# JasonTStanley/MultiDroneSim

Measured on AMD Instinct MI355X. Metric: drone-steps/sec (whole node) at N_envs×N_drones; achieved HBM GB/s vs roofline, higher is better.
Workload: dtype f32

## Files before the change

include/mds.h:

```cpp
#ifndef MDS_H
#define MDS_H

#include <stddef.h>
#include <stdint.h>

#ifdef __cplusplus
extern "C" {
#endif

#define MDS_VERSION 202
#define MDS_OBS_DIM 20
#define MDS_ACT_DIM 4
#define MDS_STATE_DIM 13
#define MDS_DES_DIM 11
#define MDS_LEM_DIM 7
#define MDS_GEO_AUX_DIM 13

typedef enum mds_status {
  MDS_OK = 0,
  MDS_EINVAL = -1,
  MDS_ENOMEM = -2,
  MDS_EHIP = -3,
  MDS_EALIGN = -4,
  MDS_ESTATE = -5,
// ... 34 lines not shown
const char* mds_last_error(void);

int mds_default_config(int drone_model, mds_config* cfg);
int mds_default_geometric_gains(mds_geometric_gains* gains);

int mds_create(const mds_config* cfg, mds_handle** out);
int mds_destroy(mds_handle* h);

int mds_get_derived(const mds_handle* h, double out[8]);

int mds_reset(mds_handle* h, const double* xyz_host, const double* rpy_host, void* stream);

int mds_state_ptrs(mds_handle* h, void* comp_dev[13], size_t stride_elems[13], void* origin_dev[3]);

int mds_get_state(mds_handle* h, double* state_host, void* stream);
int mds_set_state(mds_handle* h, const double* state_host, void* stream);

int mds_set_origin(mds_handle* h, const double* origin_host, void* stream);

int mds_get_obs(mds_handle* h, void* obs_dev, void* stream);

int mds_step(mds_handle* h, const void* action_dev, void* obs_dev, void* stream);

int mds_set_wind(mds_handle* h, const double force_world[3]);

#define MDS_SEG_DIM 40
int mds_set_trajectory_segments(mds_handle* h, const double* segs_host, const int32_t* offsets_host,
                                const int32_t* compound_host, const double* anchor_host, int32_t total_segments, void* stream);
int mds_traj_eval(mds_handle* h, double t, void* des_dev, void* stream);

int mds_set_lemniscate(mds_handle* h, const double* params_host, void* stream);
int mds_traj_yaw_free(mds_handle* h);
int mds_set_traj_specialisation(mds_handle* h, int on);
int mds_set_geometric_gains(mds_handle* h, const mds_geometric_gains* gains);

int mds_step_geometric(mds_handle* h, double t, void* obs_dev, void* action_dev, void* stream);

int mds_rollout_geometric(mds_handle* h, double t0, int n_steps, void* obs_dev, int obs_every_step, void* stream);

int mds_rollout_step(mds_handle* h, const void* actions_dev, int n_action_sets, int first_step, int n_steps, void* obs_log_dev,
                     int log_slots, int episode_len, void* stream);
int mds_rollout_step_fused(mds_handle* h, const void* actions_dev, int n_action_sets, int first_step, int n_steps, void* obs_log_dev,
                           int log_slots, int episode_len, int steps_per_launch, void* stream);
int mds_reset_async(mds_handle* h, void* stream);

typedef struct mds_episode_params {
  int32_t max_steps;
  int32_t reserved;
  double z_min, z_max, max_dist, max_tilt, max_speed, max_rate;
  double reward_r0, term_penalty;
} mds_episode_params;
int mds_default_episode_params(mds_episode_params* params);
int mds_set_episodes(mds_handle* h, const mds_episode_params* params, const double* target_host, void* stream);
int mds_rollout_episodes(mds_handle* h, const void* actions_dev, int n_action_sets, int first_step, int n_steps, void* obs_log_dev,
                         int log_slots, void* reward_log_dev, int32_t* flags_log_dev, int steps_per_launch, void* obs_dev, void* stream);
int mds_step_episodes(mds_handle* h, const void* action_dev, void* obs_dev, void* final_obs_dev, void* reward_dev, int32_t* flags_dev,
                      void* stream);
int mds_episode_ptrs(mds_handle* h, void* ptrs[5]);

#define MDS_EPISODE_MAX_OBSTACLES 16
typedef struct mds_episode_safety {
  double safety_radius, zscale;
  int32_t n_obs, reserved;
} mds_episode_safety;
int mds_set_episode_safety(mds_handle* h, const mds_episode_safety* params, const double* obstacles_host, void* stream);
int mds_episode_safety_ptrs(mds_handle* h, void* ptrs[2]);
// ... 137 lines not shown
```

multidronesim_amd/_capi.py:

```python
from __future__ import annotations

import ctypes as C
import os

_HERE = os.path.dirname(os.path.abspath(__file__))
LIB_PATH = os.environ.get("MDS_LIB_PATH") or os.path.join(_HERE, "libmds.so")

MDS_OK = 0
MDS_F32, MDS_F64, MDS_F16, MDS_F32C = 0, 1, 2, 3
MDS_PHYSICS_DYN, MDS_PHYSICS_DYN_DRAG, MDS_PHYSICS_DYN_GND, MDS_PHYSICS_DYN_DW, MDS_PHYSICS_DYN_GND_DRAG_DW = 0, 1, 2, 3, 4
MDS_INTEGRATOR_EULER, MDS_INTEGRATOR_RK4 = 0, 1
MDS_CF2X, MDS_CF2P = 0, 1
OBS_DIM, ACT_DIM, STATE_DIM, DES_DIM, LEM_DIM, GEO_AUX_DIM, SEG_DIM = 20, 4, 13, 11, 7, 13, 40


class MdsConfig(C.Structure):
    _fields_ = [("num_envs", C.c_int32), ("num_drones", C.c_int32), ("dtype", C.c_int32), ("physics", C.c_int32),
                ("integrator", C.c_int32), ("drone_model", C.c_int32), ("pyb_freq", C.c_int32),
                ("ctrl_freq", C.c_int32), ("device", C.c_int32), ("track_last_rpm", C.c_int32),
                ("M", C.c_double), ("L", C.c_double), ("KF", C.c_double), ("KM", C.c_double), ("J", C.c_double * 3),
                ("G", C.c_double), ("thrust2weight", C.c_double), ("drag_coeff", C.c_double * 3)]


class MdsGeometricGains(C.Structure):
# ... 26 lines not shown
class MdsEpisodeRandomisation(C.Structure):
    _fields_ = [("seed", C.c_uint64), ("first_env", C.c_int64)] + [(k, C.c_double * 3) for k in ("pos", "rpy", "vel", "rate")]


class MdsError(RuntimeError):
    def __init__(self, status, where, detail):
        super().__init__(f"{where}: {detail} (mds_status {status})")
        self.status = status


_P = C.c_void_p
_PD = C.POINTER(C.c_double)

PROTOTYPES = {
    "mds_version": (C.c_int, []),
    "mds_strerror": (C.c_char_p, [C.c_int]),
    "mds_last_error": (C.c_char_p, []),
    "mds_default_config": (C.c_int, [C.c_int, C.POINTER(MdsConfig)]),
    "mds_default_geometric_gains": (C.c_int, [C.POINTER(MdsGeometricGains)]),
    "mds_create": (C.c_int, [C.POINTER(MdsConfig), C.POINTER(_P)]),
    "mds_destroy": (C.c_int, [_P]),
    "mds_get_derived": (C.c_int, [_P, _PD]),
    "mds_reset": (C.c_int, [_P, _PD, _PD, _P]),
    "mds_state_ptrs": (C.c_int, [_P, C.POINTER(C.c_void_p), C.POINTER(C.c_size_t), C.POINTER(C.c_void_p)]),
    "mds_get_state": (C.c_int, [_P, _PD, _P]),
    "mds_set_state": (C.c_int, [_P, _PD, _P]),
    "mds_set_origin": (C.c_int, [_P, _PD, _P]),
    "mds_get_obs": (C.c_int, [_P, _P, _P]),
    "mds_step": (C.c_int, [_P, _P, _P, _P]),
    "mds_set_wind": (C.c_int, [_P, _PD]),
    "mds_set_lemniscate": (C.c_int, [_P, _PD, _P]),
    "mds_traj_yaw_free": (C.c_int, [_P]),
    "mds_set_traj_specialisation": (C.c_int, [_P, C.c_int]),
    "mds_set_trajectory_segments": (C.c_int, [_P, _PD, C.POINTER(C.c_int32), C.POINTER(C.c_int32), _PD, C.c_int32, _P]),
    "mds_traj_eval": (C.c_int, [_P, C.c_double, _P, _P]),
    "mds_set_geometric_gains": (C.c_int, [_P, C.POINTER(MdsGeometricGains)]),
    "mds_step_geometric": (C.c_int, [_P, C.c_double, _P, _P, _P]),
    "mds_rollout_geometric": (C.c_int, [_P, C.c_double, C.c_int, _P, C.c_int, _P]),
    "mds_set_rollout_streams": (C.c_int, [_P, C.c_int]),
    "mds_get_last_rollout_streams": (C.c_int, [_P]),
    "mds_rollout_streams_for": (C.c_int, [_P, C.c_int, C.c_int]),
    "mds_set_rollout_form": (C.c_int, [_P, C.c_int, C.c_int]),
    "mds_rollout_form_for": (C.c_int, [_P, C.c_int]),
    "mds_get_last_rollout_form": (C.c_int, [_P]),
    "mds_rollout_step": (C.c_int, [_P, _P, C.c_int, C.c_int, C.c_int, _P, C.c_int, C.c_int, _P]),
    "mds_rollout_step_fused": (C.c_int, [_P, _P, C.c_int, C.c_int, C.c_int, _P, C.c_int, C.c_int, C.c_int, _P]),
    "mds_reset_async": (C.c_int, [_P, _P]),
    "mds_default_episode_params": (C.c_int, [C.POINTER(MdsEpisodeParams)]),
    "mds_set_episodes": (C.c_int, [_P, C.POINTER(MdsEpisodeParams), _PD, _P]),
    "mds_rollout_episodes": (C.c_int, [_P, _P, C.c_int, C.c_int, C.c_int, _P, C.c_int, _P, _P, C.c_int, _P, _P]),
    "mds_step_episodes": (C.c_int, [_P, _P, _P, _P, _P, _P, _P]),
    "mds_episode_ptrs": (C.c_int, [_P, C.POINTER(C.c_void_p)]),
    "mds_set_episode_safety": (C.c_int, [_P, C.POINTER(MdsEpisodeSafety), _PD, _P]),
    "mds_episode_safety_ptrs": (C.c_int, [_P, C.POINTER(C.c_void_p)]),
    "mds_set_episode_randomisation": (C.c_int, [_P, C.POINTER(MdsEpisodeRandomisation), _P]),
    "mds_reset_episodes": (C.c_int, [_P, _P, _P]),
    "mds_rollout_geometric_fused": (C.c_int, [_P, C.c_double, C.c_int, _P, _P, _P]),
    "mds_lemniscate_eval": (C.c_int, [_P, C.c_double, _P, _P]),
    "mds_geometric_compute": (C.c_int, [_P, _P, _P, _P, _P, _P]),
    "mds_input_to_action": (C.c_int, [_P, _P, _P, _P]),
    "mds_action_to_input": (C.c_int, [_P, _P, C.c_int, _P, _P]),
    "mds_obs_to_model": (C.c_int, [_P, _P, C.c_int, _P, _P]),
    "mds_quadrotor_dynamics": (C.c_int, [C.c_int, C.c_int, _P, _P, C.c_double, _PD, C.c_double, _P, _P]),
    "mds_compare_models": (C.c_int, [_P, C.c_int, _P, _PD, _PD, C.c_double, C.c_double, _PD, C.c_double, _P, _P, _P, _P]),
    "mds_linear_xdot": (C.c_int, [_P, C.c_int, _P, _P, _PD, _PD, C.c_double, _P, _P]),
    "mds_rpy_to_rot": (C.c_int, [C.c_int, C.c_int, _P, _P, _P]),
# ... 102 lines not shown
```

multidronesim_amd/csrc/mds_api.hip:

```cpp
#include <hip/hip_runtime.h>
#include <math.h>
#include <stdio.h>
#include <stdlib.h>
#include <string.h>

#include <new>
#include <type_traits>
#include <unordered_map>
#include <vector>

#include "../../include/mds.h"
#include "mds_consts.hpp"
#include "mds_devmem.hpp"
#include "mds_kernels.hip"
#include "mds_traj_image.hpp"
#ifndef MDS_PART
#define MDS_PART 3
#endif
#if MDS_PART & 1
#include "mds_episode_kernels.hip"
#endif
#if MDS_PART & 2
#include "mds_cbf_kernels.hip"
#include "mds_fedce_kernels.hip"
// ... 73 lines not shown


}

template <typename T> struct HostParams {
  Consts<T> c;
  EnvFx<T> fx;
  CbfParams<T> cbf;
  DslPidGains<T> pid;
  LqrGain<T> lqr;
  LqrYoGain<T> lqr_yo;
  Lqr12Gain<T> lqr12;
};

struct mds_handle {
  explicit mds_handle(const DevAllocator& a) : mem(a) {}
  DevMem mem;
  mds_config cfg = {};
  mds_geometric_gains gains = {};
  double wind[3] = {0.0, 0.0, 0.0};
  int n = 0;
  size_t ld = 0;
  void* state = nullptr;
  void* state_lo = nullptr;
  void* origin = nullptr;
  void* last_rpm = nullptr;
  void* lem = nullptr;
  double* scratch = nullptr;
  double* init_pose = nullptr;
  bool has_traj = false;
  int traj_mode = 0;
  bool traj_yaw_free = false;
  bool traj_spec = true;
  double* segs = nullptr;
  int nseg_total = 0;
  int* tinfo = nullptr;
  HostParams<float> p32 = {};
  HostParams<double> p64 = {};
  bool has_cbf = false;
  mds_cbf_params cbf = {};
  int* pair_ij = nullptr;
  void* obstacles = nullptr;
  int* cbf_order = nullptr;
  int* cbf_count = nullptr;
  int cbf_calls_half[2] = {-1, -1};
  int* cbf_cost = nullptr;
  int cbf_calls = -1;
  int rollout_streams = 0;
  hipStream_t split_st = nullptr;
  hipEvent_t split_ev[2] = {nullptr, nullptr};
  int last_rollout_streams = 0;
  int rollout_form = 0;
  int rollout_chunk = 50;
  int last_rollout_form = 0;
  bool next_nom_ok[3] = {false, false, false};
  double next_nom_t[3] = {0.0, 0.0, 0.0};
  bool cbf_hildreth = false;
  bool cbf_q4 = false;
  int cbf_last_step_kernel = -1;
  bool cbf_step_persistent = false;
  bool cbf_fused = false;
  void* cbf_unom = nullptr;
  void* cbf_xdes = nullptr;
  void* cbf_usafe = nullptr;
  void* ll = nullptr;
  void* pid = nullptr;
// ... 586 lines not shown

int step_env_ctrl(mds_handle* h, int ctrl, double t, const void* u_in, double thrust_offset, void* obs, void* act, hipStream_t st) {
  const dim3 grid = grid_for(h->n, kBlock);
  const int K = h->cfg.pyb_freq / h->cfg.ctrl_freq, D = h->cfg.num_drones;
  void* rpm = rpm_track(h);
  void* abuf = K > 1 ? h->act_scratch : nullptr;
  const void* gain = ctrl == 1 ? h->gain_dev[0] : nullptr;
  with_dtype_no_half(h->cfg.dtype, [&](auto DT) {
    using T = typename decltype(DT)::T;
    with_int<0, 1, 2, 3>(ctrl, [&](auto CTRL) {
      with_flags([&](auto DRAG) {
        k_step_ctrl_env<T, T, DRAG(), CTRL()><<<grid, kBlock, 0, st>>>(params<T>(h).c, params<T>(h).fx, gain, h->n, h->ld, D, t, h->traj_mode,
                                                                       (const T*)h->state, (T*)h->state_alt, (const T*)h->origin, (const T*)h->lem,
                                                                       SegTable{h->segs, h->nseg_total}, h->tinfo, (T*)rpm, (T*)h->ll, (const T*)u_in,
                                                                       (T)(1.0 / h->cfg.ctrl_freq), (T)thrust_offset, (T*)abuf, (T*)obs, (T*)act, K == 1);
      }, has_drag(h));
    });
  });
  MDS_HIP(hipGetLastError());
  void* home = h->state;
  void* tmp = h->state; h->state = h->state_alt; h->state_alt = tmp;
  if (K > 1) return step_env_plain(h, h->act_scratch, obs, st, 1, home);
  return envfx_return_home(h, home, st);
}

int mds_step(mds_handle* h, const void* action, void* obs, void* stream) {
  MDS_DEV(h);
  if (!h || !action) return fail(MDS_EINVAL, "mds_step: null argument");
  if (!aligned16(action) || !aligned16(obs)) return fail(MDS_EALIGN, "mds_step: action_dev/obs_dev");
  if (int rc = step_plain(h, action, obs, Chain{(hipStream_t)stream, 0, 0})) return rc;
  return check_launches();
}

int mds_set_lemniscate(mds_handle* h, const double* params, void* stream) {
  MDS_DEV(h);
  if (!h || !params) return fail(MDS_EINVAL, "mds_set_lemniscate: null argument");
  hipStream_t st = (hipStream_t)stream;
  const int n = h->n;
  double* centres = new (std::nothrow) double[(size_t)n * 3];
  if (!centres) return fail(MDS_ENOMEM, "mds_set_lemniscate: host allocation");
  bool yaw_free = true;
  for (int i = 0; i < n; ++i) {
    for (int k = 0; k < 3; ++k) centres[(size_t)3 * i + k] = params[(size_t)7 * i + 2 + k];
    yaw_free = yaw_free && params[(size_t)7 * i + 5] == 0.0;
  }
  int rc = mds_set_origin(h, centres, stream);
  delete[] centres;
  if (rc != MDS_OK) return rc;
  MDS_HIP(hipMemcpyAsync(h->scratch, params, (size_t)n * 7 * sizeof(double), hipMemcpyHostToDevice, st));
  with_dtype(h->cfg.dtype, [&](auto DT) {
    using T = typename decltype(DT)::T;
    k_set_planes<T><<<grid_for(n, 256), 256, 0, st>>>(n, h->ld, 7, h->scratch, (T*)h->lem);
  });
  MDS_HIP(hipGetLastError());
  MDS_HIP(hipStreamSynchronize(st));
  h->has_traj = true;
  h->traj_mode = 1;
  h->traj_yaw_free = yaw_free;
  return MDS_OK;
}

int mds_traj_yaw_free(mds_handle* h) { return h && h->traj_yaw_free ? 1 : 0; }

int mds_set_traj_specialisation(mds_handle* h, int on) {
  if (!h) return fail(MDS_EINVAL, "mds_set_traj_specialisation: null handle");
  h->traj_spec = on != 0;
  return MDS_OK;
}

static bool use_yaw_free(const mds_handle* h) { return h->traj_mode == 1 && h->traj_yaw_free && h->traj_spec; }

int mds_set_trajectory_segments(mds_handle* h, const double* segs, const int32_t* offsets, const int32_t* compound,
                                const double* anchor, int32_t total, void* stream) {
  MDS_DEV(h);
  if (!h || !segs || !offsets || !compound || !anchor) return fail(MDS_EINVAL, "mds_set_trajectory_segments: null argument");
  const int n = h->n;
  std::vector<int> ti;
  std::vector<double> fm;
  int nu = 0;
  const char* why = "";
  const int brc = build_traj_image(segs, offsets, compound, n, total, fm, ti, nu, &why);
  if (brc != MDS_OK) return fail(brc, why);
  if (int rc = h->mem.alloc(&h->tinfo, sizeof(int) * 3 * n)) return rc;
  const int rc = h->mem.replace(&h->segs, sizeof(double) * fm.size(), [&](void* new_segs) -> int {
    MDS_HIP(hipMemcpy(new_segs, fm.data(), sizeof(double) * fm.size(), hipMemcpyHostToDevice));
    if (int orc = mds_set_origin(h, anchor, stream)) return orc;
    MDS_HIP(hipMemcpy(h->tinfo, ti.data(), sizeof(int) * 3 * n, hipMemcpyHostToDevice));
    return MDS_OK;
  });
  if (rc != MDS_OK) return rc;
  h->nseg_total = nu;
  h->has_traj = true;
  h->traj_mode = 2;
  h->traj_yaw_free = false;
  return MDS_OK;
}

int mds_traj_eval(mds_handle* h, double t, void* des, void* stream) {
  MDS_DEV(h);
  if (!h || !des) return fail(MDS_EINVAL, "mds_traj_eval: null argument");
  if (h->traj_mode == 1) return mds_lemniscate_eval(h, t, des, stream);
  if (h->traj_mode != 2) return fail(MDS_ESTATE, "mds_traj_eval: no trajectories set");
  hipStream_t st = (hipStream_t)stream;
  with_dtype(h->cfg.dtype, [&](auto DT) {
    using S = typename decltype(DT)::S;
    k_traj_eval<S><<<grid_for(h->n, 256), 256, 0, st>>>(h->n, t, SegTable{h->segs, h->nseg_total}, h->tinfo, (S*)des);
  });
  MDS_HIP(hipGetLastError());
  return MDS_OK;
}

int mds_set_geometric_gains(mds_handle* h, const mds_geometric_gains* g) {
  if (!h || !g) return fail(MDS_EINVAL, "mds_set_geometric_gains: null argument");
  if (!(g->max_tilt_angle > 0) || !(g->max_tilt_angle < M_PI / 2)) return fail(MDS_EINVAL, "mds_set_geometric_gains: max_tilt_angle");
  h->gains = *g;
  refill_consts(h);
  return MDS_OK;
}

int mds_set_wind(mds_handle* h, const double force_world[3]) {
  if (!h || !force_world) return fail(MDS_EINVAL, "mds_set_wind: null argument");
  for (int k = 0; k < 3; ++k) h->wind[k] = force_world[k];
  refill_consts(h);
  return MDS_OK;
}

static int step_geometric(mds_handle* h, double t, void* obs, void* act, const Chain& ch) {
// ... 6 lines not shown
  const bool rk4 = h->cfg.integrator == MDS_INTEGRATOR_RK4, drag = has_drag(h);
  if (h->traj_mode == 2) {
    with_flags([&](auto RK4, auto DRAG) {
      with_dtype(h->cfg.dtype, [&](auto DT) {
        using T = typename decltype(DT)::T; using S = typename decltype(DT)::S;
        k_step_traj<T, S, RK4(), DRAG(), DT.COMP><<<grid, kBlock, pad, st>>>(params<T>(h).c, h->n, h->ld, t, (S*)h->state, (const T*)h->origin,
                                                                             SegTable{h->segs, h->nseg_total}, h->tinfo, (T*)rpm_track(h), (S*)obs,
                                                                             (S*)act, (int)batch0, (S*)h->state_lo);
      });
    }, rk4, drag);
    return MDS_OK;
  }
  with_flags([&](auto Y0, auto HAS_OBS, auto HAS_ACT, auto RK4, auto DRAG) {
    with_dtype(h->cfg.dtype, [&](auto DT) {
      using T = typename decltype(DT)::T; using S = typename decltype(DT)::S;
      auto* const k = Y0() ? &k_step_geometric_y0<T, S, HAS_OBS(), HAS_ACT(), RK4(), DRAG(), DT.COMP>
                           : &k_step_geometric<T, S, HAS_OBS(), HAS_ACT(), RK4(), DRAG(), DT.COMP>;
      k<<<grid, kBlock, pad, st>>>(params<T>(h).c, h->n, h->ld, t, (S*)h->state, (const T*)h->lem, (T*)rpm_track(h), (S*)obs, (S*)act, (int)batch0,
                                   (S*)h->state_lo);
    });
  }, use_yaw_free(h), obs != nullptr, act != nullptr, rk4, drag);
  return MDS_OK;
}

int mds_step_geometric(mds_handle* h, double t, void* obs, void* act, void* stream) {
  MDS_DEV(h);
  if (!h) return fail(MDS_EINVAL, "mds_step_geometric: null handle");
  if (!h->has_traj) return fail(MDS_ESTATE, "mds_step_geometric: call mds_set_lemniscate first");
  if (!aligned16(obs) || !aligned16(act)) return fail(MDS_EALIGN, "mds_step_geometric: obs_dev/action_dev");
  if (int rc = step_geometric(h, t, obs, act, Chain{(hipStream_t)stream, 0, 0})) return rc;
  return check_launches();
}

static void launch_rollout_kernel(mds_handle* h, int ctrl, double t0, int n_steps, void* obs_log, size_t log_stride, void* obs_last, hipStream_t st) {
  const dim3 grid = grid_for(h->n, kBlock);
  const double dt = 1.0 / h->cfg.ctrl_freq;
  const int omode = obs_log == nullptr ? kObsLast : log_stride == 0 ? kObsInPlace : kObsLog;
  auto launch = [&](auto DT, auto CTRL) {
    using T = typename decltype(DT)::T; using S = typename decltype(DT)::S;
    constexpr int COMP = DT.COMP ? 1 : 0;
    const void* gain = nullptr;
    if constexpr (CTRL() >= 1) gain = h->gain_dev[CTRL() - 1];
    with_flags([&](auto RK4, auto DRAG) {
      auto roll = [&](auto OBS) {
        if (h->traj_mode == 2) {
          if constexpr (CTRL() <= 1)
            k_rollout_traj<T, S, RK4(), DRAG(), CTRL(), COMP, OBS()><<<grid, kBlock, 0, st>>>(
                params<T>(h).c, gain, h->n, h->ld, t0, dt, n_steps, (S*)h->state, (const T*)h->origin, SegTable{h->segs, h->nseg_total}, h->tinfo,
                (T*)rpm_track(h), (S*)obs_log, log_stride, (S*)obs_last, (S*)h->state_lo);
        } else {
          auto* k = &k_rollout_geometric<T, S, RK4(), DRAG(), CTRL(), COMP, OBS()>;
          if constexpr (CTRL() == 0)
            if (use_yaw_free(h)) k = &k_rollout_geometric_y0<T, S, RK4(), DRAG(), COMP, OBS()>;
          k<<<grid, kBlock, 0, st>>>(params<T>(h).c, gain, h->n, h->ld, t0, dt, n_steps, (S*)h->state, (const T*)h->lem, (T*)rpm_track(h), (S*)obs_log,
                                     log_stride, (S*)obs_last, (T*)h->ll, (const S*)obs_last, (S*)h->state_lo);
        }
      };
      constexpr bool kPerObs = sizeof(T) == 4 && !RK4() && !DRAG() && CTRL() == 0;
      if constexpr (kPerObs) with_int<kObsInPlace, kObsLog, kObsLast>(omode, roll);
      else roll(std::integral_constant<int, -1>{});
    }, h->cfg.integrator == MDS_INTEGRATOR_RK4, has_drag(h));
  };
  if (ctrl >= 2) with_int<2, 3>(ctrl, [&](auto CTRL) { with_dtype_no_half(h->cfg.dtype, [&](auto DT) { launch(DT, CTRL); }); });
  else with_int<1, 0>(ctrl, [&](auto CTRL) { with_dtype(h->cfg.dtype, [&](auto DT) { launch(DT, CTRL); }); });
}

int mds_rollout_geometric(mds_handle* h, double t0, int n_steps, void* obs, int obs_every_step, void* stream) {
  MDS_DEV(h);
  if (!h || n_steps < 0) return fail(MDS_EINVAL, "mds_rollout_geometric");
  if (!h->has_traj) return fail(MDS_ESTATE, "mds_rollout_geometric: call mds_set_lemniscate first");
  if (!aligned16(obs)) return fail(MDS_EALIGN, "mds_rollout_geometric: obs_dev");
  hipStream_t st = (hipStream_t)stream;
  const double dt = 1.0 / h->cfg.ctrl_freq;
  if (rollout_form_policy(h, n_steps) == 2) {
    h->last_rollout_streams = 1;
    h->last_rollout_form = 2;
    for (Chunks c{n_steps, h->rollout_chunk, t0, dt, 0, 0}; c.k < n_steps; c.advance(c.len())) {
      const bool last = c.k + c.len() == n_steps;
      launch_rollout_kernel(h, 0, c.t, c.len(), obs_every_step ? obs : nullptr, 0, (!obs_every_step && last) ? obs : nullptr, st);
    }
    return check_launches();
  }
  if (!h->envfx) h->last_rollout_form = 1;
  double t = t0;
// ... 1707 lines not shown
```

multidronesim_amd/csrc/mds_kernels.hip:

```cpp
#include <hip/hip_runtime.h>
#include <type_traits>

#include "mds_math.hpp"
#include "mds_traj.hpp"

namespace mds {

typedef _Float16 half_t;

constexpr int kBlock = 256;
constexpr int kWave = 64;
constexpr int kStepMinWaves = 4;

#if defined(__HIP_DEVICE_COMPILE__)
#define MDS_KEEP_V(x) asm volatile("" : "+v"(x))
#define MDS_KEEP_S(x) asm volatile("" : "+s"(x))
#else
#define MDS_KEEP_V(x) ((void)0)
#define MDS_KEEP_S(x) ((void)0)
#endif
#if defined(__HIP_DEVICE_COMPILE__) || defined(__HIPCC__)
#define MDS_CONST_AS __attribute__((address_space(4)))
#else
#define MDS_CONST_AS
// ... 600 lines not shown
    if (state_lo) store_resid<S, T>(state_lo, ld, i, r);
  }
}

template <typename T, typename S>
__global__ void k_lqr12_compute(const Consts<T> c, const Lqr12Gain<T> K, const int n, const S* __restrict__ obs,
                                const S* __restrict__ des, S* __restrict__ u_out, S* __restrict__ act_out) {
  const int i = blockIdx.x * blockDim.x + threadIdx.x;
  if (i >= n) return;
  const S* o = obs + (size_t)i * 20;
  const S* d = des + (size_t)i * 11;
  T u[4], act[4];
  const V3<T> perr = {(T)o[0] - (T)d[0], (T)o[1] - (T)d[1], (T)o[2] - (T)d[2]};
  lqr12_control<T>(c, K, obs_rpy<T>(o), obs_ang_vel<T>(o), obs_vel<T>(o), perr, V3<T>{(T)d[3], (T)d[4], (T)d[5]}, (T)d[9], (T)d[10], u);
  input_to_action(c, u, act);
  if (u_out) store4<S, T>(u_out + (size_t)i * 4, u);
  if (act_out) store4<S, T>(act_out + (size_t)i * 4, act);
}

template <typename S>
__global__ void k_traj_eval(const int n, const double t, const SegTable segs, const int* __restrict__ tinfo,
                            S* __restrict__ des) {
  const int i = blockIdx.x * blockDim.x + threadIdx.x;
  if (i >= n) return;
  double d11[11];
  traj_eval(segs, traj_info(tinfo, i), t, d11);
  for (int k = 0; k < 11; ++k) des[(size_t)i * 11 + k] = (S)d11[k];
}

constexpr int kObsLast = 0, kObsInPlace = 1, kObsLog = 2;
template <typename T, bool RK4, bool DRAG, int CTRL, int COMP, int OBS> constexpr int rollout_min_waves() {
  return !(sizeof(T) == 4 && !RK4 && !DRAG && CTRL == 0 && COMP == 0) ? 1 : (OBS == kObsInPlace || OBS == kObsLog) ? 6 : OBS == kObsLast ? 5 : 1;
}
template <typename T, typename S, bool RK4, bool DRAG, int CTRL, int COMP, int OBS, bool Y0>
__device__ __forceinline__ void rollout_geometric_body(
    unsigned char* lds, const Consts<T>& c_arg, const void* __restrict__ Kp, const int n, const size_t ld, double t, const double ctrl_dt,
    const int n_steps, S* __restrict__ state, const T* __restrict__ lem, T* __restrict__ last_rpm, S* __restrict__ obs_log,
    const size_t log_stride, S* __restrict__ obs_last, T* __restrict__ ll, const S* __restrict__ obs_prev, S* __restrict__ state_lo) {
  static_assert(!Y0 || CTRL == 0, "the yaw-free form is GeometricControl's");
  const bool comp = COMP < 0 ? state_lo != nullptr : COMP != 0;
  const int omode = OBS < 0 ? (obs_log == nullptr ? kObsLast : log_stride == 0 ? kObsInPlace : kObsLog) : OBS;
  constexpr bool kLean = !RK4 && COMP != 1;
  const int i = blockIdx.x * kBlock + threadIdx.x;
  const bool valid = i < n;
  if (n <= 0) return;
  const size_t il = (size_t)min(i, n - 1);
  GeoIn<T> in;
  resid_zero(in.r);
  if (comp) load_resid<S, T>(state_lo, ld, il, in.r);
  T prev[4] = {T(0), T(0), T(0), T(0)};
  T thr[4] = {T(0), T(0), T(0), T(0)};
  LowLevelState<T> L;
  L.last_omega = L.integral = {T(0), T(0), T(0)};
  load_geo_in<T, S>(state, lem, ld, il, in);
  if (DRAG)
    for (int k = 0; k < 4; ++k) prev[k] = last_rpm[k * ld + il];
  if (CTRL >= 2) {
    L = load_lowlevel(ll, ld, il);
    if (CTRL == 3) load4<S, T>(obs_prev + il * kObsDim + 16, thr);
  }
  constexpr bool kCarry = CTRL == 0 && OBS != kObsLast;
  Frame<T> F;
  if (kCarry) F = make_frame(in.s.q, in.s.w);
  ObsRowOffs row_offs = obs_row_offs<S, true>(i, threadIdx.x);
  ObsRowOffs* const ro = OBS != kObsLast ? &row_offs : nullptr;
  for (int k = 0; k < n_steps; ++k) {
    T o[kObsDim];
    const bool last = k == n_steps - 1;
    const bool want = omode != kObsLast || (obs_last != nullptr && last);
#if defined(__HIP_DEVICE_COMPILE__)
    const Consts<T> MDS_CONST_AS* cp = (const Consts<T> MDS_CONST_AS*)__builtin_amdgcn_kernarg_segment_ptr();
    MDS_KEEP_S(cp);
    const Consts<T> c = kLean ? load_const(cp) : c_arg;
#else
    const Consts<T>& c = c_arg;
#endif
    T act[4], clipped[4];
    {
      if (kLean) {
        MDS_KEEP_V(in.P.a);
        if (!Y0) MDS_KEEP_V(in.P.yaw_rate);
      }
      const Desired<T> des = lemniscate_local<T, Y0>(in.P, t);
      T u[4];
      if (CTRL == 0) {
        if (!kCarry) {
          F = make_frame(in.s.q, in.s.w);
        } else if (kLean) {
          MDS_KEEP_V(F.r22m1);
          F.R.m[8] = T(1) + F.r22m1;
        }
        geometric_control<T, Y0>(c, in.s.p - des.p, F.R, in.s.v, F.av, des, u, nullptr);
      } else if (CTRL == 1) {
        lqr12_control<T>(c, *static_cast<const Lqr12Gain<T>*>(Kp), euler_from_quat(in.s.q), quat_rotate(in.s.q, in.s.w), in.s.v, in.s.p - des.p,
                         des.v, des.yaw, des.yaw_rate, u);
      } else if (CTRL == 2) {
        lqr_omega_control<T>(c, *static_cast<const LqrGain<T>*>(Kp), euler_from_quat(in.s.q), in.s.v, in.s.p, des.p, des.v, des.yaw, u);
      } else {
        lqr_yank_omega_control<T>(c, *static_cast<const LqrYoGain<T>*>(Kp), euler_from_quat(in.s.q), thr, in.s.v, in.s.p, des.p, des.v,
                                  des.yaw, u);
      }
      if (CTRL <= 1) input_to_action(c, u, act);
      else if (CTRL == 2) thrust_omega_control(c, (T)ctrl_dt, u, in.s.w, L, act);
      else yank_omega_control(c, (T)ctrl_dt, u, thr, in.s.w, L, act);
    }
    if (comp) aviary_step_comp<T, RK4, DRAG>(c, in.s, in.r, act, prev, clipped);
    else if (CTRL == 0) aviary_step<T, RK4, DRAG>(c, in.s, F, act, prev, clipped);
    else aviary_step<T, RK4, DRAG>(c, in.s, act, prev, clipped);
    if (CTRL == 3)
      for (int j = 0; j < 4; ++j) thr[j] = clipped[j];
    if (kCarry) {
      F = make_frame(in.s.q, in.s.w);
      if (want) pack_obs(in.s, F, V3<T>{in.P.cx, in.P.cy, in.P.cz}, clipped, o);
    } else if (want) {
      pack_obs(in.s, V3<T>{in.P.cx, in.P.cy, in.P.cz}, clipped, o);
    }
    if (valid && last && (DRAG || last_rpm)) {
      unsigned iu = (unsigned)i;
      MDS_KEEP_V(iu);
      for (int j = 0; j < 4; ++j) *lane_ptr(last_rpm + j * ld, iu) = DRAG ? prev[j] : clipped[j];
    }
    if (omode == kObsInPlace) write_obs_rows<S, T, true, kLean>(lds, obs_log, n, i, valid, o, ro);
    else if (omode == kObsLog) write_obs_rows<S, T, false, kLean>(lds, obs_log + (size_t)k * log_stride, n, i, valid, o, ro);
    if (omode != kObsInPlace && obs_last != nullptr && last) write_obs_rows<S, T, false, kLean>(lds, obs_last, n, i, valid, o, ro);
    t = uniform_f64(t + ctrl_dt);
  }
  if (valid) {
    store_state<S, T>(state, ld, i, in.s);
    if (comp) store_resid<S, T>(state_lo, ld, i, in.r);
    if (DRAG && n_steps <= 0)
      for (int k = 0; k < 4; ++k) last_rpm[k * ld + i] = prev[k];
    if (CTRL >= 2) store_lowlevel(ll, ld, i, L);
  }
}
template <typename T, typename S, bool RK4, bool DRAG, int CTRL = 0, int COMP = -1, int OBS = -1>
__global__ __launch_bounds__(kBlock, (rollout_min_waves<T, RK4, DRAG, CTRL, COMP, OBS>())) void k_rollout_geometric(
    const Consts<T> c_arg, const void* __restrict__ Kp, const int n, const size_t ld, double t, const double ctrl_dt, const int n_steps,
    S* __restrict__ state, const T* __restrict__ lem, T* __restrict__ last_rpm, S* __restrict__ obs_log, const size_t log_stride,
    S* __restrict__ obs_last, T* __restrict__ ll = nullptr, const S* __restrict__ obs_prev = nullptr, S* __restrict__ state_lo = nullptr) {
  __shared__ __align__(16) unsigned char lds[kBlock * kObsDim * sizeof(S)];
  rollout_geometric_body<T, S, RK4, DRAG, CTRL, COMP, OBS, false>(lds, c_arg, Kp, n, ld, t, ctrl_dt, n_steps, state, lem, last_rpm, obs_log,
                                                                  log_stride, obs_last, ll, obs_prev, state_lo);
}
template <typename T, typename S, bool RK4, bool DRAG, int COMP = -1, int OBS = -1>
__global__ __launch_bounds__(kBlock, (rollout_min_waves<T, RK4, DRAG, 0, COMP, OBS>())) void k_rollout_geometric_y0(
    const Consts<T> c_arg, const void* __restrict__ Kp, const int n, const size_t ld, double t, const double ctrl_dt, const int n_steps,
    S* __restrict__ state, const T* __restrict__ lem, T* __restrict__ last_rpm, S* __restrict__ obs_log, const size_t log_stride,
    S* __restrict__ obs_last, T* __restrict__ ll = nullptr, const S* __restrict__ obs_prev = nullptr, S* __restrict__ state_lo = nullptr) {
  __shared__ __align__(16) unsigned char lds[kBlock * kObsDim * sizeof(S)];
  rollout_geometric_body<T, S, RK4, DRAG, 0, COMP, OBS, true>(lds, c_arg, Kp, n, ld, t, ctrl_dt, n_steps, state, lem, last_rpm, obs_log,
                                                              log_stride, obs_last, ll, obs_prev, state_lo);
}

template <typename T, typename S, bool RK4, bool DRAG, int CTRL, int COMP = -1, int OBS = -1>
__global__ __launch_bounds__(kBlock) void k_rollout_traj(const Consts<T> c, const void* __restrict__ Kp, const int n, const size_t ld, double t,
                                                         const double ctrl_dt, const int n_steps, S* __restrict__ state,
                                                         const T* __restrict__ origin, const SegTable segs,
                                                         const int* __restrict__ tinfo, T* __restrict__ last_rpm,
                                                         S* __restrict__ obs_log, const size_t log_stride, S* __restrict__ obs_last,
                                                         S* __restrict__ state_lo = nullptr) {
  __shared__ __align__(16) unsigned char lds[kBlock * kObsDim * sizeof(S)];
  const bool comp = COMP < 0 ? state_lo != nullptr : COMP != 0;
  const int omode = OBS < 0 ? (obs_log == nullptr ? kObsLast : log_stride == 0 ? kObsInPlace : kObsLog) : OBS;
  const int i = blockIdx.x * kBlock + threadIdx.x;
  const bool valid = i < n;
  State<T> s;
  Resid<T> r;
  resid_zero(r);
  if (valid && comp) load_resid<S, T>(state_lo, ld, i, r);
  V3<T> org = {T(0), T(0), T(0)};
  TrajInfo ti = {0, 1, 0, 0};
  T prev[4] = {T(0), T(0), T(0), T(0)};
  if (valid) {
    load_state<S, T>(state, ld, i, s);
    org = load_origin(origin, ld, i);
    ti = traj_info(tinfo, i);
    load_prev_rpm<DRAG>(last_rpm, ld, i, prev);
  }
  for (int k = 0; k < n_steps; ++k) {
    T o[kObsDim];
    const bool last = k == n_steps - 1;
    const bool want = omode != kObsLast || (obs_last != nullptr && last);
    if (valid) {
      const Desired<T> des = TrajLocal<T>::eval(segs, ti, t, org);
// ... 567 lines not shown
```

multidronesim_amd/csrc/mds_math.hpp:

```cpp
#pragma once
#include <math.h>
#include <stdint.h>

#if defined(__HIPCC__)
#define MDS_HD __host__ __device__ __forceinline__
#else
#define MDS_HD inline
#endif

namespace mds {

#if defined(__HIP_DEVICE_COMPILE__)
MDS_HD float m_rcp(float x) { return __builtin_amdgcn_rcpf(x); }
MDS_HD float m_sqrt(float x) { return __builtin_amdgcn_sqrtf(x); }
MDS_HD float m_rsqrt(float x) { return __builtin_amdgcn_rsqf(x); }
#else
MDS_HD float m_rcp(float x) { return 1.0f / x; }
MDS_HD float m_sqrt(float x) { return sqrtf(x); }
MDS_HD float m_rsqrt(float x) { return 1.0f / sqrtf(x); }
#endif
MDS_HD double m_rcp(double x) { return 1.0 / x; }
MDS_HD double m_sqrt(double x) { return sqrt(x); }
MDS_HD double m_rsqrt(double x) { return 1.0 / sqrt(x); }
MDS_HD float m_fma(float a, float b, float c) { return fmaf(a, b, c); }
// ... 591 lines not shown
      step_rk4_comp<T, DRAG>(c, s, r, clipped, drag_s);
    } else {
      T thrust;
      V3<T> tau;
      rotor_wrench(c, clipped, &thrust, &tau);
      step_euler_wrench_comp<T, DRAG>(c, s, r, thrust, tau, drag_s);
    }
    if (DRAG)
      for (int i = 0; i < 4; ++i) rpm_prev[i] = clipped[i];
  }
}

template <typename T> MDS_HD void pack_obs(const State<T>& s, const Frame<T>& F, V3<T> origin, const T rpm[4], T o[20]) {
  const V3<T> av = F.av;
  const V3<T> rpy = rpy_from_rot(F.R, s.q);
  o[0] = s.p.x + origin.x; o[1] = s.p.y + origin.y; o[2] = s.p.z + origin.z;
  o[3] = s.q[0]; o[4] = s.q[1]; o[5] = s.q[2]; o[6] = s.q[3];
  o[7] = rpy.x; o[8] = rpy.y; o[9] = rpy.z;
  o[10] = s.v.x; o[11] = s.v.y; o[12] = s.v.z;
  o[13] = av.x; o[14] = av.y; o[15] = av.z;
  o[16] = rpm[0]; o[17] = rpm[1]; o[18] = rpm[2]; o[19] = rpm[3];
}
template <typename T> MDS_HD void pack_obs(const State<T>& s, V3<T> origin, const T rpm[4], T o[20]) {
  pack_obs(s, make_frame(s.q, s.w), origin, rpm, o);
}

template <typename T> struct Desired {
  V3<T> p, v, a;
  T yaw, yaw_rate;
};
template <typename T> struct LemniscateParams {
  T a, omega, cx, cy, cz, yaw_rate, phase_shift;
};
template <typename T, bool Y0 = false> MDS_HD Desired<T> lemniscate_local(const LemniscateParams<T>& P, double t) {
  Desired<T> d;
  const T th = reduced_phase<T>(t, P.omega, P.phase_shift);
  T s, c;
  m_sincos(th, &s, &c);
  const T s2 = s * s, c2 = c * c;
  const T den = T(1) + s2;
  const T inv = m_rcp(den);
  const T inv2 = inv * inv;
  const T aw = P.a * P.omega;
  d.p = {P.a * s * c * inv, P.a * c * inv, T(0)};
  d.v = {-aw * (s2 * s2 + s2 + (s2 - T(1)) * c2) * inv2, -aw * s * (s2 + T(2) * c2 + T(1)) * inv2, T(0)};
  const T sin2 = T(2) * s * c, cos2 = c2 - s2, cos4 = T(1) - T(2) * sin2 * sin2;
  const T inv3 = T(-0.125) * (inv2 * inv);
  const T aw2 = aw * P.omega;
  d.a = {T(4) * aw2 * sin2 * (T(3) * cos2 + T(7)) * inv3, aw2 * c * (T(44) * cos2 + cos4 - T(21)) * inv3, T(0)};
  if (Y0) {
    d.yaw = d.yaw_rate = T(0);
    return d;
  }
  T sy = T(0), cy = T(1);
  if (P.yaw_rate != T(0)) {
    const T ph = reduced_phase<T>(t, P.yaw_rate, T(0));
    m_sincos(ph, &sy, &cy);
  }
  d.yaw = T(3.14159265358979323846) * sy;
  d.yaw_rate = T(3.14159265358979323846) * P.yaw_rate * cy;
  return d;
}

template <typename T> MDS_HD void input_to_action(const Consts<T>& c, const T u_in[4], T rpm[4]) {
  const T u0 = m_max(u_in[0], T(0));
  const T a = T(0.25) * u0, b1 = u_in[1] * c.inv_2L, b2 = u_in[2] * c.inv_2L, d = u_in[3] * c.inv_4r;
  T th[4] = {a - b2 - d, a + b1 + d, a + b2 - d, a - b1 + d};
  for (int i = 0; i < 4; ++i) {
    th[i] = m_clamp(th[i], c.min_motor_thrust, c.max_motor_thrust);
    rpm[i] = m_sqrt(th[i] * c.inv_kf);
  }
}
template <typename T> MDS_HD void action_to_input(const Consts<T>& c, const T action[4], int cap_rpm, T u[4]) {
  T r[4];
  for (int i = 0; i < 4; ++i) r[i] = cap_rpm ? m_clamp(action[i], T(0), c.max_rpm) : action[i];
  u[0] = c.kf * ((r[0] * r[0] + r[1] * r[1]) + (r[2] * r[2] + r[3] * r[3]));
  u[1] = c.arm_kf * ((r[1] - r[3]) * (r[1] + r[3]));
  u[2] = c.arm_kf * ((r[2] - r[0]) * (r[2] + r[0]));
  u[3] = c.km * ((r[1] - r[0]) * (r[1] + r[0]) + (r[3] - r[2]) * (r[3] + r[2]));
}

template <typename T> struct GeoAux {
  T force;
  V3<T> w_des;
  V3<T> b1d, b2d, b3d;
};
template <typename T, bool Y0 = false>
MDS_HD void geometric_control(const Consts<T>& c, V3<T> p_rel, const M3<T>& R, V3<T> v_world, V3<T> w,
                              const Desired<T>& des, T u[4], GeoAux<T>* aux) {
  const V3<T> Kp = {c.kp[0], c.kp[1], c.kp[2]}, Kv = {c.kv[0], c.kv[1], c.kv[2]};
  const V3<T> v_b = mulT(R, v_world);
  V3<T> RTvd, tw;
  if (Y0) {
    RTvd = {m_fma(R.m[0], des.v.x, R.m[3] * des.v.y), m_fma(R.m[1], des.v.x, R.m[4] * des.v.y), m_fma(R.m[2], des.v.x, R.m[5] * des.v.y)};
// ... 350 lines not shown
```

multidronesim_amd/envs/BaseAviary.py:

```python
from __future__ import annotations

import ctypes as C
import time

import numpy as np
import torch

from .. import _capi as capi
from .._device import DTYPE_BY_NAME, TORCH_DTYPE, default_device_index, forget_env_device, note_env_device, require_gpu, stream_ptr, to_device
from ..utils.enums import DroneModel, Physics

__all__ = ["BaseAviary", "DroneModel", "Physics"]

_PHYSICS_MAP = {Physics.DYN: capi.MDS_PHYSICS_DYN, Physics.PYB: capi.MDS_PHYSICS_DYN,
                Physics.PYB_DRAG: capi.MDS_PHYSICS_DYN_DRAG, Physics.PYB_GND: capi.MDS_PHYSICS_DYN_GND,
                Physics.PYB_DW: capi.MDS_PHYSICS_DYN_DW, Physics.PYB_GND_DRAG_DW: capi.MDS_PHYSICS_DYN_GND_DRAG_DW}
_MODEL_MAP = {DroneModel.CF2X: capi.MDS_CF2X, DroneModel.CF2P: capi.MDS_CF2P}
_PYB_SUBSTITUTED = (Physics.PYB, Physics.PYB_DRAG, Physics.PYB_GND, Physics.PYB_DW, Physics.PYB_GND_DRAG_DW)
_CONSTANT_KEYS = {"M": 1, "L": 1, "KF": 1, "KM": 1, "J": 3, "G": 1, "thrust2weight": 1, "drag_coeff": 3}


def apply_constants(cfg, constants):
    for key, val in (constants or {}).items():
        if key not in _CONSTANT_KEYS:
# ... 431 lines not shown
        for name, val in (("pos", pos), ("rpy", rpy), ("vel", vel), ("rate", rate)):
            setattr(p, name, (C.c_double * 3)(*np.broadcast_to(np.asarray(val, dtype=np.float64), (3,))))
        capi.check(self._lib.mds_set_episode_randomisation(self._h, C.byref(p), self._stream()), "mds_set_episode_randomisation")

    def reset_episodes(self):
        self._require_open()
        capi.check(self._lib.mds_reset_episodes(self._h, C.c_void_p(self._obs.data_ptr()), self._stream()), "mds_reset_episodes")
        return self._obs

    def set_rollout_streams(self, n_streams: int = 0):
        self._require_open()
        capi.check(self._lib.mds_set_rollout_streams(self._h, C.c_int(int(n_streams))), "mds_set_rollout_streams")

    def last_rollout_streams(self) -> int:
        self._require_open()
        return int(self._lib.mds_get_last_rollout_streams(self._h))

    def rollout_streams_for(self, n_steps: int, cbf: bool = False) -> int:
        self._require_open()
        return int(self._lib.mds_rollout_streams_for(self._h, C.c_int(1 if cbf else 0), C.c_int(int(n_steps))))

    def set_rollout_form(self, form: int = 0, steps_per_launch: int = 0):
        self._require_open()
        capi.check(self._lib.mds_set_rollout_form(self._h, C.c_int(int(form)), C.c_int(int(steps_per_launch))), "mds_set_rollout_form")

    def traj_yaw_free(self) -> bool:
        self._require_open()
        return bool(self._lib.mds_traj_yaw_free(self._h))

    def set_traj_specialisation(self, on: bool = True):
        self._require_open()
        capi.check(self._lib.mds_set_traj_specialisation(self._h, C.c_int(1 if on else 0)), "mds_set_traj_specialisation")

    def rollout_form_for(self, n_steps: int) -> int:
        self._require_open()
        return int(self._lib.mds_rollout_form_for(self._h, C.c_int(int(n_steps))))

    def last_rollout_form(self) -> int:
        self._require_open()
        return int(self._lib.mds_get_last_rollout_form(self._h))

    def rollout_geometric_fused(self, t0: float, n_steps: int, log: bool = False, log_out: torch.Tensor | None = None,
                                controller: str = "geometric"):
        self._require_open()
        if log and log_out is None:
            log_out = torch.empty((n_steps, self.NUM_ENVS, self.NUM_DRONES, capi.OBS_DIM), dtype=self.dtype, device=self.device)
        fn = {"lqr": self._lib.mds_rollout_lqr_fused, "geometric": self._lib.mds_rollout_geometric_fused,
              "nominal": self._lib.mds_rollout_nominal_fused}[controller]
        capi.check(fn(self._h, C.c_double(t0), C.c_int(n_steps), C.c_void_p(log_out.data_ptr() if log_out is not None else None),
                      C.c_void_p(self._obs.data_ptr()), self._stream()), "mds_rollout_*_fused")
        self.step_counter += n_steps * self.PYB_STEPS_PER_CTRL
        return self._obs, log_out

    def set_dslpid_gains(self, ctrl):
        from ..control.DSLPIDControl import gains_struct
        capi.check(self._lib.mds_set_dslpid_gains(self._h, C.byref(gains_struct(ctrl))), "mds_set_dslpid_gains")

    def step_dslpid(self, target_pos, target_rpy, return_action: bool = False):
        self._require_open()
        def prep(a):
            if not isinstance(a, torch.Tensor):
                a = np.asarray(a, dtype=np.float64)
                if a.shape == (self.NUM_DRONES, 3):
                    a = np.broadcast_to(a, (self.NUM_ENVS, self.NUM_DRONES, 3))
            return to_device(a, self.device, self.dtype).reshape(self.n, 3)
        tp, tr = prep(target_pos), prep(target_rpy)
# ... 121 lines not shown
```

Measured before the change: 80.84 billion.

## Precompute lemniscate phase sin/cos table for periodic yaw-free geometric rollouts

When lemniscate parameters repeat every 64 drones, a small kernel builds a table of per-step, per-lane sin/cos values of the trajectory phase. A new rollout kernel variant loads these from the table instead of running reduced_phase and sincos every step. The table is kept across calls and reused when the next rollout continues from the stored time. The aim is to take transcendental work out of the inner step loop. In exchange it adds an extra table-build launch, a global load per step, and cached state that has to stay consistent with the rollout time.

```diff
diff --git a/include/mds.h b/include/mds.h
--- a/include/mds.h
+++ b/include/mds.h
@@ -90,6 +90,9 @@
 int mds_set_lemniscate(mds_handle* h, const double* params_host, void* stream);
 int mds_traj_yaw_free(mds_handle* h);
 int mds_set_traj_specialisation(mds_handle* h, int on);
+int mds_traj_phase_periodic(mds_handle* h);
+int mds_set_traj_phase_table(mds_handle* h, int on);
+int mds_get_last_rollout_phase_table(mds_handle* h);
 int mds_set_geometric_gains(mds_handle* h, const mds_geometric_gains* gains);
 
 int mds_step_geometric(mds_handle* h, double t, void* obs_dev, void* action_dev, void* stream);
diff --git a/multidronesim_amd/_capi.py b/multidronesim_amd/_capi.py
--- a/multidronesim_amd/_capi.py
+++ b/multidronesim_amd/_capi.py
@@ -82,6 +82,9 @@
     "mds_set_lemniscate": (C.c_int, [_P, _PD, _P]),
     "mds_traj_yaw_free": (C.c_int, [_P]),
     "mds_set_traj_specialisation": (C.c_int, [_P, C.c_int]),
+    "mds_traj_phase_periodic": (C.c_int, [_P]),
+    "mds_set_traj_phase_table": (C.c_int, [_P, C.c_int]),
+    "mds_get_last_rollout_phase_table": (C.c_int, [_P]),
     "mds_set_trajectory_segments": (C.c_int, [_P, _PD, C.POINTER(C.c_int32), C.POINTER(C.c_int32), _PD, C.c_int32, _P]),
     "mds_traj_eval": (C.c_int, [_P, C.c_double, _P, _P]),
     "mds_set_geometric_gains": (C.c_int, [_P, C.POINTER(MdsGeometricGains)]),
diff --git a/multidronesim_amd/csrc/mds_api.hip b/multidronesim_amd/csrc/mds_api.hip
--- a/multidronesim_amd/csrc/mds_api.hip
+++ b/multidronesim_amd/csrc/mds_api.hip
@@ -129,6 +129,14 @@
   int traj_mode = 0;
   bool traj_yaw_free = false;
   bool traj_spec = true;
+  bool traj_phase_periodic = false;
+  bool phase_tab_on = true;
+  void* phase_tab = nullptr;
+  bool phase_tab_filled = false;
+  int phase_tab_rows = 0;
+  int phase_tab_row = 0;
+  double phase_tab_t = 0.0;
+  int last_rollout_phase_table = 0;
   double* segs = nullptr;
   int nseg_total = 0;
   int* tinfo = nullptr;
@@ -781,6 +789,12 @@
   return check_launches();
 }
 
+constexpr int kPhaseTabRows = 2048;
+static bool phase_table_built(const mds_handle* h) {
+  return h->cfg.dtype == MDS_F32 && h->cfg.integrator != MDS_INTEGRATOR_RK4 && !has_drag(h) && !h->envfx;
+}
+static size_t phase_table_bytes(const mds_handle* h) { return (size_t)kPhaseTabRows * kPhaseLanes * 2 * comp_size(h->cfg.dtype); }
+
 int mds_set_lemniscate(mds_handle* h, const double* params, void* stream) {
   MDS_DEV(h);
   if (!h || !params) return fail(MDS_EINVAL, "mds_set_lemniscate: null argument");
@@ -793,6 +807,12 @@
     for (int k = 0; k < 3; ++k) centres[(size_t)3 * i + k] = params[(size_t)7 * i + 2 + k];
     yaw_free = yaw_free && params[(size_t)7 * i + 5] == 0.0;
   }
+  const bool phase_periodic = lemniscate_phase_periodic(params, n);
+  if (yaw_free && phase_periodic && phase_table_built(h))
+    if (int arc = h->mem.alloc(&h->phase_tab, phase_table_bytes(h))) {
+      delete[] centres;
+      return arc;
+    }
   int rc = mds_set_origin(h, centres, stream);
   delete[] centres;
   if (rc != MDS_OK) return rc;
@@ -806,16 +826,27 @@
   h->has_traj = true;
   h->traj_mode = 1;
   h->traj_yaw_free = yaw_free;
+  h->traj_phase_periodic = phase_periodic;
+  h->phase_tab_filled = false;
   return MDS_OK;
 }
 
 int mds_traj_yaw_free(mds_handle* h) { return h && h->traj_yaw_free ? 1 : 0; }
+int mds_traj_phase_periodic(mds_handle* h) { return h && h->traj_phase_periodic ? 1 : 0; }
 
 int mds_set_traj_specialisation(mds_handle* h, int on) {
   if (!h) return fail(MDS_EINVAL, "mds_set_traj_specialisation: null handle");
   h->traj_spec = on != 0;
   return MDS_OK;
 }
+
+int mds_set_traj_phase_table(mds_handle* h, int on) {
+  if (!h) return fail(MDS_EINVAL, "mds_set_traj_phase_table: null handle");
+  h->phase_tab_on = on != 0;
+  return MDS_OK;
+}
+
+int mds_get_last_rollout_phase_table(mds_handle* h) { return h ? h->last_rollout_phase_table : 0; }
 
 static bool use_yaw_free(const mds_handle* h) { return h->traj_mode == 1 && h->traj_yaw_free && h->traj_spec; }
 
@@ -842,6 +873,7 @@
   h->has_traj = true;
   h->traj_mode = 2;
   h->traj_yaw_free = false;
+  h->traj_phase_periodic = false;
   return MDS_OK;
 }
 
@@ -914,10 +946,32 @@
   return check_launches();
 }
 
+static const float* phase_table_rows(mds_handle* h, double t0, double dt, int n_steps, hipStream_t st) {
+  using T = float;
+  const bool continues = h->phase_tab_filled && memcmp(&t0, &h->phase_tab_t, sizeof(double)) == 0;
+  if (!continues || h->phase_tab_row + n_steps > h->phase_tab_rows) {
+    const int rows = continues ? std::min(kPhaseTabRows, std::max(2 * h->phase_tab_rows, n_steps)) : n_steps;
+    k_lemniscate_phase_table<T><<<grid_for((size_t)rows * kPhaseLanes, 256), 256, 0, st>>>(h->n, h->ld, t0, dt, rows, (const T*)h->lem, (T*)h->phase_tab);
+    h->phase_tab_filled = true;
+    h->phase_tab_rows = rows;
+    h->phase_tab_row = 0;
+  }
+  const T* first = (const T*)h->phase_tab + (size_t)h->phase_tab_row * kPhaseLanes * 2;
+  h->phase_tab_row += n_steps;
+  for (int k = 0; k < n_steps; ++k) t0 += dt;
+  h->phase_tab_t = t0;
+  return first;
+}
+static bool use_phase_table(const mds_handle* h, int n_steps, hipStream_t st) {
+  return use_yaw_free(h) && h->traj_phase_periodic && h->phase_tab_on && h->phase_tab && n_steps >= 1 && n_steps <= kPhaseTabRows &&
+         !stream_is_capturing(st);
+}
+
 static void launch_rollout_kernel(mds_handle* h, int ctrl, double t0, int n_steps, void* obs_log, size_t log_stride, void* obs_last, hipStream_t st) {
   const dim3 grid = grid_for(h->n, kBlock);
   const double dt = 1.0 / h->cfg.ctrl_freq;
   const int omode = obs_log == nullptr ? kObsLast : log_stride == 0 ? kObsInPlace : kObsLog;
+  h->last_rollout_phase_table = 0;
   auto launch = [&](auto DT, auto CTRL) {
     using T = typename decltype(DT)::T; using S = typename decltype(DT)::S;
     constexpr int COMP = DT.COMP ? 1 : 0;
@@ -932,6 +986,15 @@
                 (T*)rpm_track(h), (S*)obs_log, log_stride, (S*)obs_last, (S*)h->state_lo);
         } else {
           auto* k = &k_rollout_geometric<T, S, RK4(), DRAG(), CTRL(), COMP, OBS()>;
+          if constexpr (CTRL() == 0 && std::is_same_v<S, float> && !RK4() && !DRAG() && COMP == 0 && OBS() >= 0)
+            if (use_phase_table(h, n_steps, st)) {
+              const T* rows = (const T*)phase_table_rows(h, t0, dt, n_steps, st);
+              k_rollout_geometric_y0p<T, S, false, false, 0, OBS()><<<grid, kBlock, 0, st>>>(
+                  params<T>(h).c, gain, h->n, h->ld, t0, dt, n_steps, (S*)h->state, (const T*)h->lem, (T*)rpm_track(h), (S*)obs_log, log_stride,
+                  (S*)obs_last, (T*)h->ll, (const S*)obs_last, (S*)h->state_lo, rows);
+              h->last_rollout_phase_table = 1;
+              return;
+            }
           if constexpr (CTRL() == 0)
             if (use_yaw_free(h)) k = &k_rollout_geometric_y0<T, S, RK4(), DRAG(), COMP, OBS()>;
           k<<<grid, kBlock, 0, st>>>(params<T>(h).c, gain, h->n, h->ld, t0, dt, n_steps, (S*)h->state, (const T*)h->lem, (T*)rpm_track(h), (S*)obs_log,
diff --git a/multidronesim_amd/csrc/mds_kernels.hip b/multidronesim_amd/csrc/mds_kernels.hip
--- a/multidronesim_amd/csrc/mds_kernels.hip
+++ b/multidronesim_amd/csrc/mds_kernels.hip
@@ -656,12 +656,18 @@
 template <typename T, bool RK4, bool DRAG, int CTRL, int COMP, int OBS> constexpr int rollout_min_waves() {
   return !(sizeof(T) == 4 && !RK4 && !DRAG && CTRL == 0 && COMP == 0) ? 1 : (OBS == kObsInPlace || OBS == kObsLog) ? 6 : OBS == kObsLast ? 5 : 1;
 }
-template <typename T, typename S, bool RK4, bool DRAG, int CTRL, int COMP, int OBS, bool Y0>
+template <typename T> struct alignas(2 * sizeof(T)) PhaseSC {
+  T s, c;
+};
+constexpr int kPhaseLanes = kWave;
+template <typename T, typename S, bool RK4, bool DRAG, int CTRL, int COMP, int OBS, bool Y0, bool TAB = false>
 __device__ __forceinline__ void rollout_geometric_body(
     unsigned char* lds, const Consts<T>& c_arg, const void* __restrict__ Kp, const int n, const size_t ld, double t, const double ctrl_dt,
     const int n_steps, S* __restrict__ state, const T* __restrict__ lem, T* __restrict__ last_rpm, S* __restrict__ obs_log,
-    const size_t log_stride, S* __restrict__ obs_last, T* __restrict__ ll, const S* __restrict__ obs_prev, S* __restrict__ state_lo) {
+    const size_t log_stride, S* __restrict__ obs_last, T* __restrict__ ll, const S* __restrict__ obs_prev, S* __restrict__ state_lo,
+    const T* __restrict__ phase_tab = nullptr) {
   static_assert(!Y0 || CTRL == 0, "the yaw-free form is GeometricControl's");
+  static_assert(!TAB || Y0, "the phase table serves the yaw-free form");
   const bool comp = COMP < 0 ? state_lo != nullptr : COMP != 0;
   const int omode = OBS < 0 ? (obs_log == nullptr ? kObsLast : log_stride == 0 ? kObsInPlace : kObsLog) : OBS;
   constexpr bool kLean = !RK4 && COMP != 1;
@@ -688,6 +694,22 @@
   if (kCarry) F = make_frame(in.s.q, in.s.w);
   ObsRowOffs row_offs = obs_row_offs<S, true>(i, threadIdx.x);
   ObsRowOffs* const ro = OBS != kObsLast ? &row_offs : nullptr;
+  const unsigned tab_off = ((unsigned)il & (unsigned)(kPhaseLanes - 1)) * (unsigned)sizeof(PhaseSC<T>);
+  const unsigned char* tab_row = reinterpret_cast<const unsigned char*>(phase_tab);
+  auto tab_load = [&]() {
+    unsigned off = tab_off;
+    MDS_KEEP_V(off);
+    return *reinterpret_cast<const PhaseSC<T>*>(tab_row + off);
+  };
+  PhaseSC<T> sc = {T(0), T(1)};
+  if (TAB) {
+    sc = tab_load();
+    MDS_KEEP_V(sc.s);
+    MDS_KEEP_V(sc.c);
+    for (T* v : {&in.P.a, &in.P.omega, &in.P.cx, &in.P.cy, &in.P.cz, &in.s.p.x, &in.s.p.y, &in.s.p.z, &in.s.q[0], &in.s.q[1], &in.s.q[2], &in.s.q[3],
+                 &in.s.v.x, &in.s.v.y, &in.s.v.z, &in.s.w.x, &in.s.w.y, &in.s.w.z})
+      MDS_KEEP_V(*v);
+  }
   for (int k = 0; k < n_steps; ++k) {
     T o[kObsDim];
     const bool last = k == n_steps - 1;
@@ -705,7 +727,11 @@
         MDS_KEEP_V(in.P.a);
         if (!Y0) MDS_KEEP_V(in.P.yaw_rate);
       }
-      const Desired<T> des = lemniscate_local<T, Y0>(in.P, t);
+      const Desired<T> des = TAB ? lemniscate_from_sc<T, Y0>(in.P, sc.s, sc.c, t) : lemniscate_local<T, Y0>(in.P, t);
+      if (TAB) {
+        tab_row += last ? 0 : kPhaseLanes * sizeof(PhaseSC<T>);
+        sc = tab_load();
+      }
       T u[4];
       if (CTRL == 0) {
         if (!kCarry) {
@@ -739,6 +765,10 @@
     } else if (want) {
       pack_obs(in.s, V3<T>{in.P.cx, in.P.cy, in.P.cz}, clipped, o);
     }
+    if (TAB) {
+      MDS_KEEP_V(sc.s);
+      MDS_KEEP_V(sc.c);
+    }
     if (valid && last && (DRAG || last_rpm)) {
       unsigned iu = (unsigned)i;
       MDS_KEEP_V(iu);
@@ -747,7 +777,7 @@
     if (omode == kObsInPlace) write_obs_rows<S, T, true, kLean>(lds, obs_log, n, i, valid, o, ro);
     else if (omode == kObsLog) write_obs_rows<S, T, false, kLean>(lds, obs_log + (size_t)k * log_stride, n, i, valid, o, ro);
     if (omode != kObsInPlace && obs_last != nullptr && last) write_obs_rows<S, T, false, kLean>(lds, obs_last, n, i, valid, o, ro);
-    t = uniform_f64(t + ctrl_dt);
+    if (!TAB) t = uniform_f64(t + ctrl_dt);
   }
   if (valid) {
     store_state<S, T>(state, ld, i, in.s);
@@ -774,6 +804,31 @@
   __shared__ __align__(16) unsigned char lds[kBlock * kObsDim * sizeof(S)];
   rollout_geometric_body<T, S, RK4, DRAG, 0, COMP, OBS, true>(lds, c_arg, Kp, n, ld, t, ctrl_dt, n_steps, state, lem, last_rpm, obs_log,
                                                               log_stride, obs_last, ll, obs_prev, state_lo);
+}
+
+template <typename T, typename S, bool RK4, bool DRAG, int COMP = -1, int OBS = -1>
+__global__ __launch_bounds__(kBlock, (rollout_min_waves<T, RK4, DRAG, 0, COMP, OBS>())) void k_rollout_geometric_y0p(
+    const Consts<T> c_arg, const void* __restrict__ Kp, const int n, const size_t ld, double t, const double ctrl_dt, const int n_steps,
+    S* __restrict__ state, const T* __restrict__ lem, T* __restrict__ last_rpm, S* __restrict__ obs_log, const size_t log_stride,
+    S* __restrict__ obs_last, T* __restrict__ ll, const S* __restrict__ obs_prev, S* __restrict__ state_lo, const T* __restrict__ phase_tab) {
+  __shared__ __align__(16) unsigned char lds[kBlock * kObsDim * sizeof(S)];
+  rollout_geometric_body<T, S, RK4, DRAG, 0, COMP, OBS, true, true>(lds, c_arg, Kp, n, ld, t, ctrl_dt, n_steps, state, lem, last_rpm, obs_log,
+                                                                    log_stride, obs_last, ll, obs_prev, state_lo, phase_tab);
+}
+
+template <typename T>
+__global__ __launch_bounds__(256) void k_lemniscate_phase_table(const int n, const size_t ld, const double t0, const double ctrl_dt,
+                                                                const int n_rows, const T* __restrict__ lem, T* __restrict__ phase_tab) {
+  const int e = blockIdx.x * 256 + threadIdx.x, k = e / kPhaseLanes, l = e % kPhaseLanes;
+  if (n <= 0 || k >= n_rows) return;
+  const size_t i = (size_t)min(l, n - 1);
+  const T omega = lem[4 * i + 1], phase_shift = lem[4 * i + 3];
+  double t = t0;
+#pragma unroll 8
+  for (int j = 0; j < k; ++j) t = t + ctrl_dt;
+  PhaseSC<T> sc;
+  m_sincos(reduced_phase<T>(t, omega, phase_shift), &sc.s, &sc.c);
+  reinterpret_cast<PhaseSC<T>*>(phase_tab)[e] = sc;
 }
 
 template <typename T, typename S, bool RK4, bool DRAG, int CTRL, int COMP = -1, int OBS = -1>
diff --git a/multidronesim_amd/csrc/mds_math.hpp b/multidronesim_amd/csrc/mds_math.hpp
--- a/multidronesim_amd/csrc/mds_math.hpp
+++ b/multidronesim_amd/csrc/mds_math.hpp
@@ -647,11 +647,8 @@
 template <typename T> struct LemniscateParams {
   T a, omega, cx, cy, cz, yaw_rate, phase_shift;
 };
-template <typename T, bool Y0 = false> MDS_HD Desired<T> lemniscate_local(const LemniscateParams<T>& P, double t) {
+template <typename T, bool Y0 = false> MDS_HD Desired<T> lemniscate_from_sc(const LemniscateParams<T>& P, T s, T c, double t) {
   Desired<T> d;
-  const T th = reduced_phase<T>(t, P.omega, P.phase_shift);
-  T s, c;
-  m_sincos(th, &s, &c);
   const T s2 = s * s, c2 = c * c;
   const T den = T(1) + s2;
   const T inv = m_rcp(den);
@@ -675,6 +672,17 @@
   d.yaw = T(3.14159265358979323846) * sy;
   d.yaw_rate = T(3.14159265358979323846) * P.yaw_rate * cy;
   return d;
+}
+template <typename T, bool Y0 = false> MDS_HD Desired<T> lemniscate_local(const LemniscateParams<T>& P, double t) {
+  T s, c;
+  m_sincos(reduced_phase<T>(t, P.omega, P.phase_shift), &s, &c);
+  return lemniscate_from_sc<T, Y0>(P, s, c, t);
+}
+
+inline bool lemniscate_phase_periodic(const double* params, long n) {
+  for (long i = 64; i < n; ++i)
+    if (params[7 * i + 1] != params[7 * (i - 64) + 1] || params[7 * i + 6] != params[7 * (i - 64) + 6]) return false;
+  return true;
 }
 
 template <typename T> MDS_HD void input_to_action(const Consts<T>& c, const T u_in[4], T rpm[4]) {
diff --git a/multidronesim_amd/envs/BaseAviary.py b/multidronesim_amd/envs/BaseAviary.py
--- a/multidronesim_amd/envs/BaseAviary.py
+++ b/multidronesim_amd/envs/BaseAviary.py
@@ -487,6 +487,18 @@
         self._require_open()
         capi.check(self._lib.mds_set_traj_specialisation(self._h, C.c_int(1 if on else 0)), "mds_set_traj_specialisation")
 
+    def traj_phase_periodic(self) -> bool:
+        self._require_open()
+        return bool(self._lib.mds_traj_phase_periodic(self._h))
+
+    def set_traj_phase_table(self, on: bool = True):
+        self._require_open()
+        capi.check(self._lib.mds_set_traj_phase_table(self._h, C.c_int(1 if on else 0)), "mds_set_traj_phase_table")
+
+    def last_rollout_phase_table(self) -> bool:
+        self._require_open()
+        return bool(self._lib.mds_get_last_rollout_phase_table(self._h))
+
     def rollout_form_for(self, n_steps: int) -> int:
         self._require_open()
         return int(self._lib.mds_rollout_form_for(self._h, C.c_int(int(n_steps))))
```

New measurement: 83.48 billion (median of 6 runs). 3.3% higher.
